# carltonyfakhry/geneticsCRE

Measured on AMD Instinct MI355X. Metric: path_x_permutation_scores_per_sec, higher is better.
Workload: dtype u32

## Files before the change

### geneticscre_amd/csrc/gcre_host.h

```cpp
#pragma once
#include "../../include/gcre_hip.h"
#include "gcre_kernels.h"

#include <dlfcn.h>
#include <rccl/rccl.h>

#include <algorithm>
#include <array>
#include <atomic>
#include <chrono>
#include <cmath>
#include <cstdio>
#include <cstdlib>
#include <cstring>
#include <limits>
#include <memory>
#include <mutex>
#include <condition_variable>
#include <string>
#include <unordered_map>
#include <thread>
#include <functional>
#include <deque>
#include <vector>
// ... 244 lines not shown
  int meet(uint64_t tag) {
    std::vector<float> none;
    return reduce(none, tag);
  }
  void fail() {
    std::lock_guard<std::mutex> lk(m);
    failed = true;
    cv.notify_all();
  }
};

struct gcre_ctx {
  Geometry g{};
  int device = 0;
  int top_k = 12;
  hipStream_t stream = nullptr;
  hipStream_t sel_stream = nullptr;
  hipEvent_t ev_sel = nullptr, ev_sel_done = nullptr;
  bool sel_async = true;
  hipStream_t insp_stream = nullptr;
  hipEvent_t ev_insp_done = nullptr;
  hipEvent_t ev_insp_main = nullptr;
  hipEvent_t ev_tail = nullptr;
  uint32_t* d_max_tot_b = nullptr;
  std::vector<JoinPlan>* ahead = nullptr;
  bool ahead_closed = false;
  bool ahead_on = true;
  SelectState h_sel{};
  std::string err;
  int last_code = GCRE_OK;
  bool quiet = false;
  bool have_table = false, have_perms = false;
  int64_t chunk_paths = int64_t(1) << 25;
  int null_blocks_per_cu = 12;
  int cus = 256;
  int64_t overlap_launches = 0;
  int64_t stepdown_launches = 0;
  int64_t clump_launches = 0;

  uint64_t* d_case_mask = nullptr;
  uint32_t* d_masks = nullptr;
  float* d_t32 = nullptr;
  double* d_dvt = nullptr;
  double* d_dmax = nullptr;
  double* d_dmaxn = nullptr;
  uint32_t* d_null = nullptr;
  uint32_t* d_mt = nullptr;
  bool mt_stale = false;
  int ieq_batch = 0;
  int ie_quad = 1;
  int ie_flagq = 1;
  int ie_zwide = 0;
  int ie_warm_items = 4;
  int exchange_tail = 0;
  int ie_warm_segs = 1024;
  int ie_small_join_tiles = 8;
  int ie_batch = 2;
  uint32_t* d_queue = nullptr;
  uint32_t* d_max_tot = nullptr;
  uint32_t* d_ladder = nullptr;
  uint32_t g00_rows = 0xffffffffu;
  int null_kernel = 0;
  int sparse_waves_per_cu = 32;
  int ie_prune = 1;
  uint64_t mask_epoch = 0;
  uint64_t obs_epoch = 0;
  bool insp_cache = false;
  ExchangeHub* hub = nullptr;
  ncclComm_t comm = nullptr;
  int64_t rccl_calls = 0;
  DevBuf<float> d_hub_null;
  int hub_level = 0, hub_round = 0;
  int win_k0 = 0, win_K = 0;
  int win_K_nominal = 0;

  ChunkBufs scratch;
  DevBuf<uint32_t> d_sel, d_small, d_chunk, d_rec_segs;
  DevBuf<uint64_t> d_wkey, d_doff, d_scan, d_excess, d_excess_b;
  DevBuf<uint32_t> d_wcases, d_wctrls, d_wrow0, d_wrow1;
  DevBuf<uint64_t> d_ie_timing;

  struct PlaneBuf { uint32_t* p; size_t bytes; };
  std::vector<PlaneBuf> plane_pool;
  std::unordered_map<uint64_t, const gcre_pathset*> live_sets;
  std::vector<gcre_uids*> live_uids;
  std::vector<gcre_gene_tally*> live_tallies;
  gcre_gene_tally* armed_tally = nullptr;
  gcre_gene_tally* pp_tally[6] = {nullptr, nullptr, nullptr, nullptr, nullptr, nullptr};
  std::vector<gcre_exceed*> live_exceeds;
  gcre_exceed* armed_exceed = nullptr;
  gcre_exceed* pp_exceed[6] = {nullptr, nullptr, nullptr, nullptr, nullptr, nullptr};
  std::vector<gcre_hits*> live_hits;
  gcre_hits* armed_hits = nullptr;
  gcre_hits* pp_hits[6] = {nullptr, nullptr, nullptr, nullptr, nullptr, nullptr};
  int64_t hits_launches = 0;
  uint64_t next_set_id = 0;
  size_t planes_out_max = (size_t)8 << 30;

  gcre_profile prof{};
  std::vector<std::pair<hipEvent_t, hipEvent_t>> ev_null, ev_stats;
  std::vector<hipEvent_t> ev_pool;
};

struct gcre_recipe {
  uint64_t a_id = 0, z_id = 0;
  uint64_t a_ver = 0, z_ver = 0;
// ... 136 lines not shown
```

### geneticscre_amd/csrc/gcre_host.hip

```cpp
#include "gcre_host.h"

namespace {

thread_local std::string g_create_error;

inline bool poison_fresh_planes() {
  static const bool on = std::getenv("GCRE_POISON") != nullptr && std::atoi(std::getenv("GCRE_POISON")) != 0;
  return on;
}
inline void poison_planes(void* p, size_t bytes) {
  if (!poison_fresh_planes() || !p) return;
  (void)hipDeviceSynchronize();
  (void)hipMemset(p, 0x5A, bytes);
  (void)hipDeviceSynchronize();
}

inline size_t tri(size_t t) { return t * (t + 1) / 2; }

template <typename Pred>
void pack_bits_host(const int32_t* data, int64_t nrow, int ncol, bool col_major, uint64_t* out, size_t stride, Pred pred) {
  const int W = (ncol + 63) / 64;
  if (nrow <= 0 || W <= 0) return;
  unsigned T = std::min<unsigned>(16u, std::max(1u, std::thread::hardware_concurrency()));
  if (const char* e = std::getenv("GCRE_PACK_THREADS")) T = (unsigned)std::max(1, std::atoi(e));
// ... 409 lines not shown
      });
      uint32_t run = 0;
      for (size_t k = 0; k < nkeys; k++)
        for (int t = 0; t < T; t++) {
          const uint32_t h = start[(size_t)t][k];
          start[(size_t)t][k] = run;
          run += h;
        }
      run_all([&](int t) {
        const Local& L = loc[(size_t)t];
        std::vector<uint32_t>& st = start[(size_t)t];
        for (size_t e = 0; e < L.part[q].size(); e++) segs[base + st[L.key[q][e]]++] = L.part[q][e];
      });
    } else {
      std::vector<SparseSeg> all;
      all.reserve(nq);
      for (const Local& L : loc) all.insert(all.end(), L.part[q].begin(), L.part[q].end());
      auto key_of = [&](const SparseSeg& x) { return u.h_location[x.row0] + ((int64_t)x.first + first - pi[x.row0]); };
      std::stable_sort(all.begin(), all.end(), [&](const SparseSeg& x, const SparseSeg& y) { return key_of(x) < key_of(y); });
      std::copy(all.begin(), all.end(), segs.begin() + (std::ptrdiff_t)base);
    }
    base += nq;
  }
  *nscored_out = (int64_t)n_scored;
}

void build_quads_host(const gcre_uids& u, const std::vector<SparseSeg>& segs, int64_t first, int64_t nscored, int64_t n_warm,
                      std::vector<uint32_t>& quads, int64_t* quad_begin_out) {
  const auto& pi = u.h_path_idx;
  const int64_t n = (int64_t)segs.size();
  quads.clear();
  int64_t quad_begin = -1;
  const int64_t qmax = ieq_quad_segs();
  quads.reserve((size_t)n / (size_t)std::max<int64_t>(1, (qmax + 1) / 2) + 16);
  auto key_of = [&](const SparseSeg& x) { return u.h_location[x.row0] + ((int64_t)x.first + first - pi[x.row0]); };
  int64_t i = 0;
  while (i < n) {
    if (i >= n_warm && quad_begin < 0) quad_begin = (int64_t)quads.size();
    const int64_t stop = i < n_warm ? n_warm : (i < nscored ? nscored : n);
    const int64_t k0 = key_of(segs[(size_t)i]);
    const uint32_t n0 = segs[(size_t)i].n;
    int64_t j = i + 1;
    while (j < stop && j < i + qmax && segs[(size_t)j].n == n0 && key_of(segs[(size_t)j]) == k0) j++;
    quads.push_back((uint32_t)i | ((uint32_t)(j - i - 1) << 30));
    i = j;
  }
  if (quad_begin < 0) quad_begin = (int64_t)quads.size();
  *quad_begin_out = quad_begin;
}

int64_t warm_segments(const gcre_ctx* c, int64_t nseg_scored, int nkt) {
  if (c->ie_warm_segs == 0) return 0;
  const int64_t warm_min = std::max<int64_t>(256, (int64_t)c->ie_warm_segs * 8 / std::max(nkt, 8));
  return std::min<int64_t>(nseg_scored, std::min<int64_t>(std::max<int64_t>(warm_min, nseg_scored / 1024),
                                                          std::max<int64_t>(256, nseg_scored / 8)));
}

int sparse_segments(gcre_ctx* c, const gcre_uids& u, int64_t first, int64_t count, int64_t score_b, int64_t score_e,
                    int64_t plane_b, int64_t plane_e, const SparseSeg** d_out, int64_t* nsegs, int64_t* nscored,
                    gcre_uids::SegCache** entry = nullptr) {
  plane_b = std::max(plane_b, first);
  plane_e = std::min(plane_e, first + count);
  for (auto& sc : u.seg_cache)
    if (sc.first == first && sc.count == count && sc.score_b == score_b && sc.score_e == score_e && sc.plane_b == plane_b &&
        sc.plane_e == plane_e) {
      *d_out = sc.d_segs;
      *nsegs = sc.nsegs;
      *nscored = sc.nscored;
      if (entry) *entry = &sc;
      return GCRE_OK;
    }
  std::vector<SparseSeg> segs;
  int64_t n_scored_i = 0;
  gcre_uids::Prefetch* pf = u.prefetch.get();
  if (pf && pf->th.joinable()) {
    HostTimer hw("prefetched tables: wait");
    pf->th.join();
  }
  if (pf && pf->ready && pf->first == first && pf->count == count && pf->score_b == score_b && pf->score_e == score_e &&
      pf->plane_b == plane_b && pf->plane_e == plane_e) {
    segs.swap(pf->segs);
    n_scored_i = pf->nscored;
    pf->ready = false;
    pf->quads_for_table = true;
  } else {
    HostTimer ht("sparse_segments");
    build_segments_host(u, first, count, score_b, score_e, plane_b, plane_e, segs, &n_scored_i);
  }
  const size_t n_scored = (size_t)n_scored_i;
  SparseSeg* d = nullptr;
  HIP_TRY(c, hipMalloc((void**)&d, std::max<size_t>(segs.size(), 1) * sizeof(SparseSeg)));
  if (!segs.empty())
    HIP_TRY(c, hipMemcpyAsync(d, segs.data(), segs.size() * sizeof(SparseSeg), hipMemcpyHostToDevice, c->stream));
  HIP_TRY(c, hipStreamSynchronize(c->stream));
  if (u.seg_cache.size() >= 64) {
    (void)hipFree(u.seg_cache.front().d_segs);
    if (u.seg_cache.front().d_quads) (void)hipFree(u.seg_cache.front().d_quads);
    u.seg_cache.erase(u.seg_cache.begin());
  }
  u.seg_cache.push_back({first, count, score_b, score_e, plane_b, plane_e, (int64_t)segs.size(), (int64_t)n_scored, d});
  if (c->g.method == 1 && c->ie_quad) u.seg_cache.back().h_segs = std::move(segs);
  if (entry) *entry = &u.seg_cache.back();
  *d_out = d;
  *nsegs = u.seg_cache.back().nsegs;
  *nscored = (int64_t)n_scored;
  return GCRE_OK;
}
// ... 1196 lines not shown
    ia.rec_lover = r0->lover.p;
    ia.rec_slot = r0->slot.p;
    ia.rec_over = r0->over.p;
    ia.rec_planes_a = R.rec_a->d_planes;
    ia.rec_planes_z = R.rec_z->d_planes;
    ia.rec_rows_a = (uint32_t)(R.rec_a->nrows * g.method);
    ia.rec_rows_z = (uint32_t)(R.rec_z->nrows * g.method);
    ia.rec_ga = R.rec_a->plane_groups;
    ia.rec_gz = R.rec_z->plane_groups;
    if (g.method == 1) {
      HIP_TRY(c, c->d_rec_segs.reserve((size_t)std::max<int64_t>(ia.nsegs, 1) * kRecSegWords));
      HIP_TRY(c, launch_fill_rec_segs(ia.segs, ia.nsegs, r0->row0.p, r0->rowz.p, r0->linfo.p, r0->lover.p, r0->slot.p, r0->tot.p,
                                      c->d_rec_segs.p, R.st));
      ia.rec_segs = c->d_rec_segs.p;
    }
  }
  ia.t32 = c->d_t32;
  ia.d64 = c->d_dmax;
  ia.ladder = c->d_ladder;
  ia.ladder_stride = g.TD;
  ia.lad_mode = !C.scored ? 1 : (c->ie_prune ? 0 : 2);
  ia.g00_rows = c->g00_rows;
  ia.null_bits = R.w_null;
  ia.planes_out = R.res_planes ? jp.res->d_planes : nullptr;
  ia.go = R.res_planes ? jp.res->plane_groups : 0;
  ia.out_first = cb;
  ia.score_begin = (uint32_t)C.s0;
  ia.score_end = (uint32_t)C.s1;
  ia.score_segs = (uint32_t)*nseg_scored;
  ia.nkt = R.nkt_sp;
  ia.K = g.K;
  ia.mt_rows = (uint32_t)(64 * g.Wp + 1);
  ia.zoff = (uint32_t)(64 * g.Wp) << 8;
  return GCRE_OK;
}

int launch_ie_slices(JoinRun& R, const ChunkRun& C, IeArgs& ia, int planes, int64_t nseg_scored,
                     gcre_uids::SegCache* seg_entry, int64_t ie_tile_factor, bool* quad_ran) {
  gcre_ctx* c = R.c;
  const JoinPlan& jp = R.jp;
  const Geometry& g = R.g;
  hipStream_t st = R.st;
  const int64_t n = C.n;
  ia.seg_begin = 0;
  ia.seg_end = ia.nsegs;
  if (c->d_ladder && ia.lad_mode == 0) {
    int64_t n_warm = warm_segments(c, nseg_scored, R.nkt_sp);
    if (jp.exchange && R.exchanges_done < jp.exchanges && R.P > 0)
      n_warm = std::min(n_warm, std::max<int64_t>(64, (int64_t)((double)n_warm * (double)(R.se - R.sb) / (double)R.P) + 1));
    if (c->ie_warm_segs == 0) n_warm = 0;
    IeArgs wa = ia;
    wa.seg_end = n_warm;
    wa.waves_per_xcd = spread_waves(wa.waves_per_xcd, n_warm * R.nkt_sp, c->ie_warm_items);
    if (n_warm > 0) HIP_TRY(c, launch_null_ie(wa, g.method, planes, true, st));
    ia.seg_begin = n_warm;
  }
  if (ia.seg_begin >= ia.seg_end) return GCRE_OK;
  ia.queue = c->d_queue;
  ia.batch = c->ie_batch;
  bool quad = false;
  if (g.method == 1 && c->d_ladder && c->ie_quad && !ia.planes_out && seg_entry &&
      ensure_quads(c, *R.u, *seg_entry, ia.seg_begin) == GCRE_OK) {
    const int64_t nq = seg_entry->nquads - seg_entry->quad_begin;
    const int64_t qmax = ieq_quad_segs();
    quad = nq > 0 && ((ia.seg_end - ia.seg_begin) * 4 >= nq * (4 + (qmax - 1)) || c->ie_quad == 2);
    if (std::getenv("GCRE_HOST_TIMING"))
      std::fprintf(stderr, "[host] quads: %lld segments in %lld quads (%.2f per quad), %lld joined paths, quad form %s\n",
                   (long long)(ia.seg_end - ia.seg_begin), (long long)nq, (double)(ia.seg_end - ia.seg_begin) / (double)std::max<int64_t>(nq, 1),
                   (long long)n, quad ? "on" : "off");
    if (quad) {
      ia.quads = seg_entry->d_quads;
      ia.quad_begin = seg_entry->quad_begin;
      ia.quad_end = seg_entry->nquads;
      const uint64_t z_units = (uint64_t)ia.rowsz * (uint64_t)ia.gz;
      ia.flagq = (c->ie_flagq && (uint64_t)ia.mt_rows * 256u < (1ull << 31)) ? 1u : 0u;
      ia.z_wide = (c->ie_zwide || z_units >= (1ull << 22)) ? 1u : 0u;
      ia.z_tile_units = ia.z_wide ? 0u : (uint32_t)z_units;
      ia.batch = c->ieq_batch > 0 ? c->ieq_batch : std::max(1, c->ie_batch * 2);
      const int wq = std::min(c->sparse_waves_per_cu, ieq_max_waves_per_cu(planes, ia.gz, ia.rec_slot != nullptr, ia.z_wide != 0u));
      ia.waves_per_xcd = spread_waves(xcd_waves(c, wq), n * ie_tile_factor, 128);
    }
  }
  while (((ia.nsegs - ia.seg_begin) / ia.batch + 1) * (int64_t)ia.nkt > (int64_t)0xf0000000ll) ia.batch *= 2;
  const bool pruned = c->d_ladder && ia.lad_mode == 0;
  const int n_slices = (pruned && jp.exchange) ? std::max(1, jp.exchanges - R.exchanges_done) : 1;
  const int64_t r_b = quad ? ia.quad_begin : ia.seg_begin, r_e = quad ? ia.quad_end : ia.seg_end;
  int64_t lo = r_b;
  for (int sl = 0; sl < n_slices && lo < r_e; sl++) {
    int64_t hi = r_e;
    if (sl + 1 < n_slices) {
      const int m = std::min(n_slices - 1, c->exchange_tail < 0 ? n_slices / 2 : c->exchange_tail), head = n_slices - m;
      const double end = sl >= head ? (double)(sl - head + 2) / (double)(m + 1) : std::ldexp(1.0 / (double)(m + 1), -(head - 1 - sl));
      hi = std::min(r_e, std::max(lo + 1, r_b + (int64_t)((double)(r_e - r_b) * end)));
    }
    if (pruned && jp.exchange)
      if (int rc = exchange_now(R)) return rc;
    IeArgs sa2 = ia;
    if (quad) { sa2.quad_begin = lo; sa2.quad_end = hi; }
    else { sa2.seg_begin = lo; sa2.seg_end = hi; }
    HIP_TRY(c, hipMemsetAsync(sa2.queue, 0, 8 * 16 * 4, st));
    if (quad) HIP_TRY(c, launch_null_ie_quad(sa2, planes, st));
    else HIP_TRY(c, launch_null_ie(sa2, g.method, planes, c->d_ladder == nullptr, st));
    lo = hi;
  }
  if (quad) R.prof->ie_quad_launches++;
  *quad_ran = quad;
  return GCRE_OK;
// ... 67 lines not shown
    if (cb > C.sg->b || C.sg != &R.segs.front()) {
      R.recipe_broken = true;
      R.hint_broke_late = true;
    }
    if (ci) ci->inspected = false;
    *end = ChunkEnd::kRedoHint;
    return GCRE_OK;
  }
  if (ci && !C.hit) {
    std::memcpy(ci->flags, C.flags, sizeof C.flags);
    ci->flags_valid = true;
  }
  if (R.mode == kInspect) {
    if (C.sel_begun && !C.sel_done) {
      HIP_TRY(c, hipStreamSynchronize(C.sel_on));
      if (int rc = finish_selection(R, C)) return rc;
    }
    *end = ChunkEnd::kInspected;
    return GCRE_OK;
  }
  const int64_t nseg_est = std::max<int64_t>(uids_in(*R.u, cb, n), 1);
  if (c->null_kernel == 0 && C.scored && ie_dearer(g, R.nkt_sp, R.have_p0, row_max(c, jp.p0), nseg_est, n, n_list)) {
    R.res_planes_ok = false;
    *end = C.partial ? ChunkEnd::kResplit : ChunkEnd::kPricedOut;
    return GCRE_OK;
  }
  if (!C.scored && !(R.res_planes && cb < R.pl_e && cb + n > R.pl_b)) {
    *end = ChunkEnd::kNotNeeded;
    return GCRE_OK;
  }
  const int planes = counter_planes(max_tot);
  IeArgs ia{};
  int64_t nseg_scored = 0;
  gcre_uids::SegCache* seg_entry = nullptr;
  if (int rc = fill_ie_args(R, C, ia, &nseg_scored, &seg_entry)) return rc;
  R.prof->null_row_loads += ((R.have_p0 ? 0.0 : (double)row_max(c, jp.p0) * g.method * (double)nseg_est) + (double)n_list) * R.nkt_sp;
  const int wpc = std::min(c->sparse_waves_per_cu, ie_max_waves_per_cu(g.method, planes, ia.gz, ia.planes_out != nullptr, ia.rec_slot != nullptr));
  const int64_t ie_tile_factor = std::min(std::max(R.nkt_sp * c->ie_small_join_tiles / 8, 1), R.nkt_sp);
  ia.waves_per_xcd = spread_waves(xcd_waves(c, wpc), n * ie_tile_factor, 32);
  R.prof->inspect_ms += std::chrono::duration<double, std::milli>(std::chrono::steady_clock::now() - ti0).count();
  ia.stats = R.mode == kLaunch ? R.w_null + g.Kpad : R.flagblk + kFlagLookupTiles;
  if (jp.exceed || R.mode == kCount) {
    C.ie = ia;
    C.ie_planes = planes;
    C.ie_segs = nseg_scored;
    C.ie_ok = true;
    if (R.mode == kCount) {
      *end = ChunkEnd::kScored;
      return GCRE_OK;
    }
  }
  const bool timing = std::getenv("GCRE_IE_TIMING") != nullptr;
  if (timing) {
    HIP_TRY(c, c->d_ie_timing.reserve(12));
    HIP_TRY(c, hipMemsetAsync(c->d_ie_timing.p, 0, 96, st));
    ia.timing = c->d_ie_timing.p;
  }
  if (C.sel_begun && C.sel_on == st)
    if (int rc = finish_selection(R, C)) return rc;
  hipEvent_t n0 = get_event(c), n1 = get_event(c);
  bool quad = false;
  HIP_TRY(c, hipEventRecord(n0, st));
  if (int rc = launch_ie_slices(R, C, ia, planes, nseg_scored, seg_entry, ie_tile_factor, &quad)) return rc;
  HIP_TRY(c, hipEventRecord(n1, st));
  if (C.sel_begun && !C.sel_done) {
    const auto tw0 = std::chrono::steady_clock::now();
    HIP_TRY(c, hipStreamSynchronize(C.sel_on));
    R.select_wait_ms += std::chrono::duration<double, std::milli>(std::chrono::steady_clock::now() - tw0).count();
    if (int rc = finish_selection(R, C)) return rc;
  }
  if (timing && R.mode != kLaunch)
    if (int rc = print_ie_timing(R, C, ia, quad)) return rc;
  R.ev_null->emplace_back(n0, n1);
  if (C.scored) {
    R.prof->null_kernel_launches++;
    R.prof->null_alg_bytes += alg_bytes(R, cb + C.s0, C.s1 - C.s0);
  }
  R.prof->ie_launches++;
  R.prof->ie_overlap_lists += C.flags[kFlagOverlapLists];
  R.ie_stat_pending = true;
  R.ie_ran = true;
  *end = ChunkEnd::kScored;
  return GCRE_OK;
}

int score_chunk_sparse(JoinRun& R, ChunkRun& C, ChunkEnd* end) {
  gcre_ctx* c = R.c;
  const JoinPlan& jp = R.jp;
  const gcre_uids& u = *R.u;
  const Geometry& g = R.g;
  hipStream_t st = R.st;
  ChunkBufs& b = *C.b;
  ChunkInsp* ci = C.ci;
  const int64_t cb = C.cb, n = C.n;
  if (int rc = ensure_lists(c, jp.p0)) return rc;
  if (int rc = ensure_lists(c, jp.p1)) return rc;
  const uint32_t zoff = (uint32_t)(64 * g.Wp) << 8;
  const int64_t nl = n * g.method;
  HIP_TRY(c, c->d_doff.reserve((size_t)nl + 1));
  HIP_TRY(c, c->d_scan.reserve((size_t)(nl + 1023) / 1024 + 2));
  HIP_TRY(c, launch_scan_u32_u64(b.dcnt.p, nl, c->d_doff.p, c->d_scan.p, st));
  uint32_t max_tot = 0;
  uint64_t n_delta = 0;
  HIP_TRY(c, hipMemcpyAsync(&max_tot, R.flagblk + kFlagMaxTot, 4, hipMemcpyDeviceToHost, st));
  HIP_TRY(c, hipMemcpyAsync(&n_delta, c->d_doff.p + nl, 8, hipMemcpyDeviceToHost, st));
  HIP_TRY(c, hipStreamSynchronize(st));
  if (C.hit) max_tot = ci->flags[kFlagMaxTot];
  else if (ci) { ci->flags[kFlagMaxTot] = max_tot; ci->flags_valid = true; }
// ... 266 lines not shown
  return (hipGetDeviceCount(&n) == hipSuccess && n > 0) ? n : 0;
}

const char* gcre_last_error(const gcre_ctx* ctx) { return ctx ? ctx->err.c_str() : g_create_error.c_str(); }

gcre_ctx* gcre_create(int method, int n_cases, int n_ctrls, int iterations, int device) {
  if ((method != 1 && method != 2) || n_cases <= 0 || n_ctrls <= 0 || iterations < 0) {
    g_create_error = "assertion: need method in {1,2}, num_cases > 0, num_ctrls > 0, iterations >= 0";
    return nullptr;
  }
  int ndev = 0;
  if (hipGetDeviceCount(&ndev) != hipSuccess || ndev <= 0) {
    g_create_error = "no HIP device: libgcre_hip has no CPU fallback";
    return nullptr;
  }
  if (device < 0 || device >= ndev) {
    g_create_error = "device index out of range";
    return nullptr;
  }
  hipDeviceProp_t prop;
  if (hipSetDevice(device) != hipSuccess || hipGetDeviceProperties(&prop, device) != hipSuccess) {
    g_create_error = "cannot select HIP device";
    return nullptr;
  }
  if (std::strncmp(prop.gcnArchName, "gfx950", 6) != 0) {
    g_create_error = std::string("kernels are built for gfx950 only, device is ") + prop.gcnArchName;
    return nullptr;
  }
  auto* c = new gcre_ctx();
  c->device = device;
  (void)hipDeviceGetAttribute(&c->cus, hipDeviceAttributeMultiprocessorCount, device);
  Geometry& g = c->g;
  g.method = method;
  g.n = n_cases + n_ctrls;
  g.n_cases = n_cases;
  g.W = (g.n + 63) / 64;
  g.Wp = ((g.W + 3) / 4) * 4;
  g.S = g.Wp * method;
  g.K = iterations;
  g.Kpad = ((iterations + kPermTileMax - 1) / kPermTileMax) * kPermTileMax;
  g.TD = 64 * g.Wp + 1;
  c->win_k0 = 0;
  c->win_K = g.K;
  if (const char* e = std::getenv("GCRE_QUIET")) c->quiet = std::atoi(e) != 0;
  g_launch_trace = std::getenv("GCRE_LAUNCH_TRACE") != nullptr;
  if (const char* e = std::getenv("GCRE_CHUNK_PATHS")) c->chunk_paths = std::max<long long>(64, std::atoll(e));
  if (const char* e = std::getenv("GCRE_NULL_BLOCKS_PER_CU")) c->null_blocks_per_cu = std::max(1, std::atoi(e));
  if (const char* e = std::getenv("GCRE_NULL_KERNEL"))
    c->null_kernel = !std::strcmp(e, "dense") ? 1 : !std::strcmp(e, "sparse") ? 2 : !std::strcmp(e, "ie") ? 3 : 0;
  if (const char* e = std::getenv("GCRE_IE_PRUNE")) c->ie_prune = std::atoi(e) != 0;
  if (const char* e = std::getenv("GCRE_EXCHANGE_TAIL")) c->exchange_tail = std::min(std::max(std::atoi(e), -1), 64);
  if (const char* e = std::getenv("GCRE_IE_WARM")) c->ie_warm_segs = std::min(std::max(std::atoi(e), 0), 1 << 20);
  if (const char* e = std::getenv("GCRE_IE_WARM_ITEMS")) c->ie_warm_items = std::min(std::max(std::atoi(e), 1), 64);
  if (const char* e = std::getenv("GCRE_IE_SJT")) c->ie_small_join_tiles = std::atoi(e);
  if (const char* e = std::getenv("GCRE_IE_BATCH")) c->ie_batch = std::min(std::max(std::atoi(e), 1), 4096);
  if (const char* e = std::getenv("GCRE_IEQ_BATCH")) c->ieq_batch = std::max(0, std::atoi(e));
  if (const char* e = std::getenv("GCRE_IE_QUAD")) c->ie_quad = std::min(std::max(std::atoi(e), 0), 2);
  if (const char* e = std::getenv("GCRE_IE_FLAGQ")) c->ie_flagq = std::atoi(e) != 0;
  if (const char* e = std::getenv("GCRE_IE_ZWIDE")) c->ie_zwide = std::atoi(e) != 0;
  if (const char* e = std::getenv("GCRE_PLANES_OUT_MAX_MB")) c->planes_out_max = (size_t)std::max(0ll, std::atoll(e)) << 20;
  if (const char* e = std::getenv("GCRE_SPARSE_WAVES_PER_CU")) c->sparse_waves_per_cu = std::max(1, std::atoi(e));

  bool ok = hipStreamCreateWithFlags(&c->stream, hipStreamNonBlocking) == hipSuccess;
  ok = ok && hipStreamCreateWithFlags(&c->sel_stream, hipStreamNonBlocking) == hipSuccess;
  ok = ok && hipStreamCreateWithFlags(&c->insp_stream, hipStreamNonBlocking) == hipSuccess;
  ok = ok && hipEventCreateWithFlags(&c->ev_insp_done, hipEventDisableTiming) == hipSuccess;
  ok = ok && hipEventCreateWithFlags(&c->ev_insp_main, hipEventDisableTiming) == hipSuccess;
  ok = ok && hipEventCreateWithFlags(&c->ev_tail, hipEventDisableTiming) == hipSuccess;
  if (const char* e = std::getenv("GCRE_AHEAD")) c->ahead_on = std::atoi(e) != 0;
  ok = ok && hipEventCreateWithFlags(&c->ev_sel, hipEventDisableTiming) == hipSuccess;
  ok = ok && hipEventCreateWithFlags(&c->ev_sel_done, hipEventDisableTiming) == hipSuccess;
  if (const char* e = std::getenv("GCRE_SELECT_STREAM")) c->sel_async = std::atoi(e) != 0;
  ok = ok && hipMalloc((void**)&c->d_case_mask, (size_t)g.Wp * 8) == hipSuccess;
  ok = ok && hipMalloc((void**)&c->d_max_tot, kFlagWords * 4) == hipSuccess;
  ok = ok && hipMalloc((void**)&c->d_max_tot_b, kFlagWords * 4) == hipSuccess;
  ok = ok && hipMalloc((void**)&c->d_queue, 8 * 16 * 4) == hipSuccess;
  if (ok && g.Kpad > 0) {
    ok = hipMalloc((void**)&c->d_masks, (size_t)2 * g.Wp * g.Kpad * 4) == hipSuccess;
    ok = ok && hipMalloc((void**)&c->d_null, (size_t)g.Kpad * 4) == hipSuccess;
    ok = ok && hipMemsetAsync(c->d_masks, 0, (size_t)2 * g.Wp * g.Kpad * 4, c->stream) == hipSuccess;
  }
  if (ok) {
    std::vector<uint64_t> cm((size_t)g.Wp, 0);
    for (int k = 0; k < n_cases; k++) cm[(size_t)k / 64] |= uint64_t(1) << (k % 64);
    ok = hipMemcpy(c->d_case_mask, cm.data(), cm.size() * 8, hipMemcpyHostToDevice) == hipSuccess;
  }
  if (!ok) {
    g_create_error = "device allocation failed in gcre_create";
    gcre_destroy(c);
    return nullptr;
  }
  return c;
}

void gcre_destroy(gcre_ctx* c) {
  if (!c) return;
  (void)hipSetDevice(c->device);
  if (c->stream) (void)hipStreamSynchronize(c->stream);
  if (c->insp_stream) (void)hipStreamSynchronize(c->insp_stream);
  drop_ahead(c);
  while (!c->live_uids.empty()) free_uids(c->live_uids.back());
  while (!c->live_tallies.empty()) gcre_gene_tally_free(c->live_tallies.back());
  while (!c->live_exceeds.empty()) gcre_exceed_free(c->live_exceeds.back());
  while (!c->live_hits.empty()) gcre_hits_free(c->live_hits.back());
  {
    std::vector<const gcre_pathset*> sets;
// ... 1026 lines not shown
```

### geneticscre_amd/csrc/gcre_ie.hip

```cpp
#include "gcre_ie_common.h"

namespace gcre {



template <int M, int L>
__global__ __launch_bounds__(64 * kIeWaves) __attribute__((amdgpu_waves_per_eu(M == 1 ? 4 : 2))) void k_null_ie(const IeArgs a) {
  static_assert(L % 4 == 0 && L >= 8 && L <= 16, "planes come in groups of 4");
  const int lane = threadIdx.x & 63;
  const int wave = __builtin_amdgcn_readfirstlane(threadIdx.x >> 6);
  const int xcd = blockIdx.x & 7;
  const i64 wi = (i64)(blockIdx.x >> 3) * kIeWaves + wave;
  const i64 wx = a.waves_per_xcd;
  const i64 slices = 8 * wx;
  const u32 lane4 = (u32)lane * 4u;
  __shared__ u32 gmax_lds[kIeWaves][32 * 64];
  u32* scr = gmax_lds[wave] + lane;
#pragma unroll
  for (int q = 0; q < 32; q++) scr[q * 64] = 0u;

  const SparseSeg GCRE_CONSTANT* segs = (const SparseSeg GCRE_CONSTANT*)a.segs;
  const u64 GCRE_CONSTANT* loff0 = (const u64 GCRE_CONSTANT*)a.loff0;
  const u32 GCRE_CONSTANT* lidx0 = (const u32 GCRE_CONSTANT*)a.lidx0;

  int cur_kt = -1;
  __amdgpu_buffer_rsrc_t mt = __builtin_amdgcn_make_buffer_rsrc((void*)a.mt, 0, 0x7fffffff, 0x00020000);

  auto flush = [&]() {
    if (cur_kt < 0) return;
    u32* out = a.null_bits + (size_t)cur_kt * 2048 + lane * 32;
    for (int q = 0; q < 32; q++) {
      const u32 own = scr[q * 64];
      if (own != 0u) {
        atomicMax(out + q, own);
        scr[q * 64] = 0u;
      }
    }
  };

  auto to_counts = [&](const u32 (&C)[L], u32 (&R)[16]) {
#pragma unroll
    for (int l = 0; l < 16; l++) R[l] = (l < L) ? C[l] : 0u;
    transpose16(R);
  };
  auto finish_m1 = [&](const u32 (&C)[L], u32 total) {
    u32 R[16];
    to_counts(C, R);
    const u32* diag_g = (const u32*)a.t32 + sp_diag_offset(total);
    u32 v[32], o[32];
#pragma unroll
    for (int j = 0; j < 16; j++) {
      v[j] = diag_g[R[j] & 0xffffu];
      v[j + 16] = diag_g[R[j] >> 16];
    }
#pragma unroll
    for (int q = 0; q < 32; q++) o[q] = scr[q * 64];
#pragma unroll
    for (int q = 0; q < 32; q++)
      if (v[q] > o[q]) scr[q * 64] = v[q];
  };

  auto finish_m2 = [&](const u32 (&Cp)[L], const u32 (&Cn)[L], u32 tp, u32 tn) {
    u32 Rp[16], Rn[16];
    to_counts(Cp, Rp);
    to_counts(Cn, Rn);
    const double* dp = a.d64 + sp_diag_offset(tp);
    const double* dn = a.d64 + sp_diag_offset(tn);
#pragma unroll
    for (int g0 = 0; g0 < 16; g0 += 4) {
      double sp[8], sn[8];
      u32 o[8];
#pragma unroll
      for (int k = 0; k < 4; k++) {
        sp[k] = dp[Rp[g0 + k] & 0xffffu];
        sn[k] = dn[Rn[g0 + k] & 0xffffu];
        sp[k + 4] = dp[Rp[g0 + k] >> 16];
        sn[k + 4] = dn[Rn[g0 + k] >> 16];
        o[k] = scr[(g0 + k) * 64];
        o[k + 4] = scr[(g0 + k + 16) * 64];
      }
#pragma unroll
      for (int k = 0; k < 8; k++) {
        float f = (float)(sp[k] + sn[k]);
        f = (f > 0.0f) ? f : 0.0f;
        const u32 v = __float_as_uint(f);
        const int q = (k < 4) ? g0 + k : g0 + k - 4 + 16;
        if (v > o[k]) scr[q * 64] = v;
      }
    }
  };

  auto load_planes = [&](u32 (&P)[L], const u32* planes, u32 unit, int groups) {
    const u32x4* src = (const u32x4*)(planes + (u64)unit * 256u) + lane;
#pragma unroll
    for (int j = 0; j < L / 4; j++) {
      u32x4 v = {0u, 0u, 0u, 0u};
      if (j < groups) v = src[j * 64];
      P[4 * j + 0] = v.x;
      P[4 * j + 1] = v.y;
      P[4 * j + 2] = v.z;
      P[4 * j + 3] = v.w;
    }
  };

  for (int step = 0; step < a.nkt; step++) {
    const i64 item = (i64)xcd * a.nkt * wx + wi + (i64)step * wx;
    const int kt = (int)(item / slices);
    const i64 sl = item % slices;
    if (kt != cur_kt) {
      flush();
      cur_kt = kt;
      mt = __builtin_amdgcn_make_buffer_rsrc((void*)(a.mt + (size_t)kt * a.mt_rows * 64), 0, 0x7fffffff, 0x00020000);
    }
    for (i64 sidx = a.seg_begin + sl; sidx < a.seg_end; sidx += slices) {
      const u32 row0 = segs[sidx].row0;
      const u32 first = segs[sidx].first;
      const u32 npaths = segs[sidx].n;
      const u32 qv = first + (((u32)lane < npaths) ? (u32)lane : 0u);
      u32 infov[M], lovv[M];
#pragma unroll
      for (int h = 0; h < M; h++) {
        infov[h] = a.linfo[(u64)qv * M + h];
        lovv[h] = a.lover[(u64)qv * M + h];
      }
      const u32 rzv = a.rowz[qv];
      u32 zunit[M];
#pragma unroll
      for (int h = 0; h < M; h++) {
        const u32 hz = (M == 2 && (rzv >> 31)) ? (u32)(1 - h) : (u32)h;
        zunit[h] = ((u32)kt * (u32)a.rowsz + (rzv & 0x7fffffffu) * (u32)M + hz) * (u32)a.gz;
      }
      u32 ttv[M];
#pragma unroll
      for (int h = 0; h < M; h++) ttv[h] = a.tot[(u64)qv * M + h];
      u32 lv[M][8];
#pragma unroll
      for (int h = 0; h < M; h++) {
        const u32x4* lp = (const u32x4*)(a.dlist + ((u64)qv * M + h) * 8u);
        const u32x4 e0 = lp[0], e1 = lp[1];
        lv[h][0] = e0.x; lv[h][1] = e0.y; lv[h][2] = e0.z; lv[h][3] = e0.w;
        lv[h][4] = e1.x; lv[h][5] = e1.y; lv[h][6] = e1.z; lv[h][7] = e1.w;
      }

      auto stream = [&](u32 (&P)[L], const u32 GCRE_CONSTANT* list, u64 p, u64 e) {
        u32 x[16];
        for (; p + 16 <= e; p += 16) {
          load16(x, mt, lane4, *(const u32x16 GCRE_CONSTANT*)(list + p));
          add16<L>(P, x);
        }
        for (; p < e; p += 4) {
          const u32x4 offs = *(const u32x4 GCRE_CONSTANT*)(list + p);
          u32 y4[4];
#pragma unroll
          for (int j = 0; j < 4; j++) y4[j] = __builtin_amdgcn_raw_buffer_load_b32(mt, lane4, offs[j], 0);
          add4<L>(P, y4);
        }
      };

      u32 B[M][L];
#pragma unroll
      for (int h = 0; h < M; h++) {
        const u64 r = (u64)row0 * M + h;
        if (a.planes0) {
          load_planes(B[h], a.planes0, (u32)(((u64)kt * (u64)a.rows0 + r) * (u64)a.g0), a.g0);
        } else if (a.rec_slot) {
          const u32 ra = a.rec_row0[row0], rzr = a.rec_rowz[row0], rz = rzr & 0x7fffffffu, rinfo = a.rec_linfo[r];
          const u32 hz = (M == 2 && (rzr >> 31)) ? (u32)(1 - h) : (u32)h;
          u32 ZR[L], S[L];
          load_planes(B[h], a.rec_planes_a, (u32)(((u64)kt * (u64)a.rec_rows_a + (u64)ra * M + h) * (u64)a.rec_ga), a.rec_ga);
          load_planes(ZR, a.rec_planes_z, (u32)(((u64)kt * (u64)a.rec_rows_z + (u64)rz * M + hz) * (u64)a.rec_gz), a.rec_gz);
#pragma unroll
          for (int l = 0; l < L; l++) S[l] = 0u;
          const u32 rlen = linfo_len(rinfo);
          stream(S, (const u32 GCRE_CONSTANT*)(a.rec_slot + r * 8u), 0, 8);
          if (rlen > 8u) stream(S, (const u32 GCRE_CONSTANT*)(a.rec_over + a.rec_lover[r]), 0, (u64)(rlen - 8u));
          u32 cy = 0u, bw = 0u;
#pragma unroll
          for (int l = 0; l < L; l++) {
            const u32 zl = linfo_overlap(rinfo) ? ZR[l] : S[l];
            const u32 sl_ = linfo_overlap(rinfo) ? S[l] : 0u;
            const u32 s1_ = B[h][l] ^ zl ^ cy;
            cy = maj3(B[h][l], zl, cy);
            B[h][l] = s1_ ^ sl_ ^ bw;
            bw = maj3(~s1_, sl_, bw);
          }
        } else {
#pragma unroll
          for (int l = 0; l < L; l++) B[h][l] = 0u;
          stream(B[h], lidx0, loff0[r], loff0[r + 1]);
        }
      }

      for (u32 t = 0; t < npaths; t++) {
        const u32 q = first + t;
        u32 C[M][L];
#pragma unroll
        for (int h = 0; h < M; h++) {
          const u32 r0 = rdlane(infov[h], t);
          const u32 len = linfo_len(r0);
          const bool overlap = linfo_overlap(r0);
          u32 offs[8], y[8];
#pragma unroll
          for (int j = 0; j < 8; j++) offs[j] = rdlane(lv[h][j], t);
#pragma unroll
          for (int j = 0; j < 8; j++) y[j] = __builtin_amdgcn_raw_buffer_load_b32(mt, lane4, offs[j], 0);
          u32 Z[L];
          if (overlap) {
            load_planes(Z, a.planesz, rdlane(zunit[h], t), a.gz);
          } else {
#pragma unroll
            for (int l = 0; l < L; l++) Z[l] = 0u;
          }
          u32 c0, a0, c1, a1, c2, a2, d0, b0;
          csa(c0, a0, y[0], y[1], y[2]);
          csa(c1, a1, y[3], y[4], y[5]);
          csa(c2, a2, a0, a1, y[6]);
          const u32 s0 = a2 ^ y[7], c3 = a2 & y[7];
          csa(d0, b0, c0, c1, c2);
          const u32 s1 = b0 ^ c3, d1 = b0 & c3;
          u32 S[L];
          S[0] = s0; S[1] = s1; S[2] = d0 ^ d1; S[3] = d0 & d1;
#pragma unroll
          for (int l = 4; l < L; l++) S[l] = 0u;
          if (len > 8u) stream(S, (const u32 GCRE_CONSTANT*)(a.dover + rdlane(lovv[h], t)), 0, (u64)(len - 8u));
          if (overlap) {
            u32 cy = 0u, bw = 0u;
#pragma unroll
            for (int l = 0; l < L; l++) {
              const u32 s1_ = B[h][l] ^ Z[l] ^ cy;
              cy = maj3(B[h][l], Z[l], cy);
              C[h][l] = s1_ ^ S[l] ^ bw;
              bw = maj3(~s1_, S[l], bw);
            }
          } else {
            u32 cy = 0u;
#pragma unroll
            for (int l = 0; l < L; l++) {
              C[h][l] = B[h][l] ^ S[l] ^ cy;
              cy = maj3(B[h][l], S[l], cy);
            }
          }
        }
        if (a.planes_out) {
#pragma unroll
          for (int h = 0; h < M; h++) {
            const u64 rh = ((u64)a.out_first + q) * M + h;
            u32x4* dst = (u32x4*)(a.planes_out + (((u64)cur_kt * (u64)a.rows_out + rh) * (u64)a.go) * 256u) + lane;
#pragma unroll
            for (int j = 0; j < 4; j++) {
              if (j < a.go) {
                u32x4 v = {0u, 0u, 0u, 0u};
                if (4 * j < L) v = u32x4{C[h][(4 * j) % L], C[h][(4 * j + 1) % L], C[h][(4 * j + 2) % L], C[h][(4 * j + 3) % L]};
                dst[j * 64] = v;
              }
            }
          }
        }
        if (q < a.score_begin || q >= a.score_end) continue;
        if constexpr (M == 1) {
          finish_m1(C[0], rdlane(ttv[0], t));
        } else {
          finish_m2(C[0], C[M - 1], rdlane(ttv[0], t), rdlane(ttv[M - 1], t));
        }
      }
    }
  }
  flush();
}


template <int L, int GZ, bool OUT, bool REC>
__global__ __launch_bounds__(64 * kIeWaves) __attribute__((amdgpu_waves_per_eu(L <= 12 ? 4 : 3))) void k_null_ie_m1(const IeArgs a) {
  constexpr int LP = (L + 3) / 4 * 4;
  static_assert(L >= 8 && L <= 16 && GZ >= 2 && 4 * GZ <= LP, "planes come in groups of 4");
  __shared__ u32 nmax_lds[kIeWaves][32 * 64];
  const int lane = threadIdx.x & 63;
  const int wave = __builtin_amdgcn_readfirstlane(threadIdx.x >> 6);
  const u32 lane4 = (u32)lane * 4u;
  u32* nm = nmax_lds[wave] + lane;
#pragma unroll
  for (int q = 0; q < 32; q++) nm[q * 64] = 0u;
  const SparseSeg GCRE_CONSTANT* segs = (const SparseSeg GCRE_CONSTANT*)a.segs;
  const char* k_planesz = (const char*)(((u64)(u32)__builtin_amdgcn_readfirstlane((int)(u32)((u64)a.planesz >> 32)) << 32) |
                                        (u64)(u32)__builtin_amdgcn_readfirstlane((int)(u32)(u64)a.planesz));

  int cur_kt = -1;
  u32 valid = 0u;
  u32 lad_base = (a.lad_mode == 0) ? 0u : (u32)(kLadderLevels - 1 + a.lad_mode) * (u32)a.ladder_stride;
  const u32 lad_keep = (u32)kLadderLevels * (u32)a.ladder_stride;
  bool dirty = false;
  u32 n_slow = 0u;
#ifdef GCRE_IE_TIMING
  u64 tm[6] = {0, 0, 0, 0, 0, 0};
  const u64 tm_begin = __builtin_amdgcn_s_memtime();
#define GCRE_TM_MARK(var) __builtin_amdgcn_s_waitcnt(0); const u64 var = __builtin_amdgcn_s_memtime()
#define GCRE_TM_ADD(i, t1, t0) tm[i] += (t1) - (t0)
#else
#define GCRE_TM_MARK(var)
#define GCRE_TM_ADD(i, t1, t0)
#endif
  __amdgpu_buffer_rsrc_t mt = __builtin_amdgcn_make_buffer_rsrc((void*)a.mt, 0, 0x7fffffff, 0x00020000);

  auto exchange = [&]() {
    u32* out = a.null_bits + (size_t)cur_kt * 2048 + lane * 32;
    __amdgpu_buffer_rsrc_t nb = __builtin_amdgcn_make_buffer_rsrc((void*)(a.null_bits + (size_t)cur_kt * 2048), 0, 8192, 0x00020000);
    u32x4 g4[8];
#pragma unroll
    for (int j = 0; j < 8; j++) g4[j] = __builtin_amdgcn_raw_buffer_load_b128(nb, (u32)lane * 128u + (u32)j * 16u, 0, 16 );
    u32 lo = 0xffffffffu;
#pragma unroll
    for (int q = 0; q < 32; q++) {
      const u32 g = g4[q >> 2][q & 3];
      const u32 own = nm[q * 64];
      if (dirty && own > g) atomicMax(out + q, own);
      const u32 v = own > g ? own : g;
      if ((valid >> q) & 1u) lo = v < lo ? v : lo;
    }
    dirty = false;
    u32 theta = __builtin_amdgcn_readfirstlane(wave_min_u32(lo));
    if (theta == 0xffffffffu) theta = 0u;
    int j = (int)(__uint_as_float(theta) * (float)kLadderPerUnit);
    j = j < 0 ? 0 : (j > kLadderLevels - 1 ? kLadderLevels - 1 : j);
    lad_base = (u32)j * (u32)a.ladder_stride;
  };
  auto flush_tile = [&]() {
    if (cur_kt >= 0) {
      u32* out = a.null_bits + (size_t)cur_kt * 2048 + lane * 32;
#pragma unroll 8
      for (int q = 0; q < 32; q++) {
        const u32 own = nm[q * 64];
        if (own != 0u) {
          atomicMax(out + q, own);
          nm[q * 64] = 0u;
        }
      }
    }
    dirty = false;
  };

  __shared__ u32 wq_state[kIeWaves][8];
  WorkQueue wq;
  wq.st = wq_state[wave];
  wq.init(a.queue, (u32)((a.seg_end - a.seg_begin + a.batch - 1) / a.batch), (u32)a.nkt);
  {
    wq.select(blockIdx.x & 7u);
  }
  u32 ticket = wq.take(lane);
  int since = 0, period = 1;
  for (;;) {
    const u32 work = __builtin_amdgcn_readfirstlane(ticket);
    const u32 q_n = wq.get(2);
    if (work >= q_n) {
// ... 488 lines not shown
    GCRE_IE_M2(EXPR)                                               \
  }

__global__ __launch_bounds__(256) void k_fill_rec_segs(const SparseSeg* segs, i64 nsegs, const u32* r_row0, const u32* r_rowz,
                                                       const u32* r_linfo, const u32* r_lover, const u32* r_slot, const u32* r_tot,
                                                       u32* out) {
  const i64 t = (i64)blockIdx.x * blockDim.x + threadIdx.x;
  const i64 sidx = t >> 2;
  const int part = (int)(t & 3);
  if (sidx >= nsegs) return;
  const u32 row0 = segs[sidx].row0;
  u32* o = out + sidx * kRecSegWords;
  if (part == 0) {
    o[0] = r_row0[row0];
    o[1] = r_rowz[row0];
  } else if (part == 1) {
    u32 info = r_linfo[row0];
    u32 need = 3u;
    if (r_tot) {
      const u32 t = r_tot[row0];
      need = t < 16u ? 0u : (t < 256u ? 1u : (t < 4096u ? 2u : 3u));
    }
    o[2] = linfo_with_groups(info, need);
    o[3] = r_lover[row0];
  } else {
    const u32x4 v = *(const u32x4*)(r_slot + (u64)row0 * 8u + (part - 2) * 4);
    *(u32x4*)(o + 4 + (part - 2) * 4) = v;
  }
}

hipError_t launch_fill_rec_segs(const SparseSeg* segs, int64_t nsegs, const uint32_t* r_row0, const uint32_t* r_rowz,
                                const uint32_t* r_linfo, const uint32_t* r_lover, const uint32_t* r_slot, const uint32_t* r_tot,
                                uint32_t* out, hipStream_t stream) {
  if (nsegs == 0) return hipSuccess;
  const i64 blocks = (nsegs * 4 + 255) / 256;
  hipLaunchKernelGGL(k_fill_rec_segs, dim3((unsigned)blocks), dim3(256), 0, stream, segs, nsegs, r_row0, r_rowz, r_linfo, r_lover,
                     r_slot, r_tot, out);
  return hipGetLastError();
}

hipError_t launch_null_ie(const IeArgs& a, int method, int planes, bool general, hipStream_t stream) {
  const dim3 grid((unsigned)(8 * a.waves_per_xcd / kIeWaves));
  const dim3 block(64 * kIeWaves);
  if (method == 1 && !general) {
    const int gz = a.gz;
    const bool out = a.planes_out != nullptr;
    const bool rec = a.rec_slot != nullptr;
#define GCRE_LAUNCH(LL, GG, OO, RR) hipLaunchKernelGGL((k_null_ie_m1<LL, GG, OO, RR>), grid, block, 0, stream, a)
    GCRE_IE_M1(GCRE_LAUNCH)
#undef GCRE_LAUNCH
  } else if (method == 2 && !general) {
    return launch_null_ie_m2(a, planes, stream);
  } else {
#define GCRE_LAUNCH(MM, LL) hipLaunchKernelGGL((k_null_ie<MM, LL>), grid, block, 0, stream, a)
    GCRE_IE_GEN(GCRE_LAUNCH)
#undef GCRE_LAUNCH
  }
  return hipGetLastError();
}

int ie_max_waves_per_cu(int method, int planes, int gz, bool out, bool rec) {
  int blocks = 0;
  hipError_t e = hipSuccess;
  if (method == 1) {
#define GCRE_OCC(LL, GG, OO, RR) e = hipOccupancyMaxActiveBlocksPerMultiprocessor(&blocks, k_null_ie_m1<LL, GG, OO, RR>, 64 * kIeWaves, 0)
    GCRE_IE_M1(GCRE_OCC)
#undef GCRE_OCC
  } else {
    return ie2_max_waves_per_cu(planes, gz, out, rec);
  }
  if (e != hipSuccess || blocks < 1) blocks = 1;
  return blocks * kIeWaves;
}

template <int L>
__global__ __launch_bounds__(256) void k_build_planes(const u32* mt_all, u32 mt_rows, int nkt, const u64* loff,
                                                      const u32* lidx, i64 nrowhalves, int groups, u32* planes) {
  const int lane = threadIdx.x & 63;
  const i64 wave = (i64)blockIdx.x * 4 + __builtin_amdgcn_readfirstlane(threadIdx.x >> 6);
  const i64 nwaves = (i64)gridDim.x * 4;
  const u32 lane4 = (u32)lane * 4u;
  const u64 GCRE_CONSTANT* off = (const u64 GCRE_CONSTANT*)loff;
  const u32 GCRE_CONSTANT* list = (const u32 GCRE_CONSTANT*)lidx;
  const i64 items = nrowhalves * nkt;
  for (i64 it = wave; it < items; it += nwaves) {
    const i64 w = it / nrowhalves;
    const i64 rr = it - w * nrowhalves;
    __amdgpu_buffer_rsrc_t mt = __builtin_amdgcn_make_buffer_rsrc((void*)(mt_all + (size_t)w * mt_rows * 64), 0, 0x7fffffff, 0x00020000);
    u32 P[L];
#pragma unroll
    for (int l = 0; l < L; l++) P[l] = 0u;
    u64 p = off[rr];
    const u64 e = off[rr + 1];
    u32 x[16];
    for (; p + 16 <= e; p += 16) {
      load16(x, mt, lane4, *(const u32x16 GCRE_CONSTANT*)(list + p));
      add16<L>(P, x);
    }
    for (; p < e; p += 4) {
      const u32x4 offs = *(const u32x4 GCRE_CONSTANT*)(list + p);
      u32 y[4];
#pragma unroll
      for (int j = 0; j < 4; j++) y[j] = __builtin_amdgcn_raw_buffer_load_b32(mt, lane4, offs[j], 0);
      add4<L>(P, y);
    }
    u32x4* dst = (u32x4*)(planes + (((u64)w * (u64)nrowhalves + (u64)rr) * (u64)groups) * 256u) + lane;
// ... 156 lines not shown
```

Baseline: 9521 billion.

## Restructure warm IE kernel work split and merge block maxima before atomics

The general k_null_ie kernel, used for warm segments, now hands each block a contiguous chunk of segments per key tile, with one segment per wave, instead of strided slices. Its flush first reduces the per-wave LDS maxima across the block and compares them against the global null bits, so it issues fewer atomicMax operations. The warm-segment count divisor moves from 1024 to a tunable 4096, which shrinks the warm phase for large segment counts. Optional timing instrumentation is added; the kernel now uses two block barriers per flush and rejects launches where waves_per_xcd is not a multiple of kIeWaves.

```diff
diff --git a/geneticscre_amd/csrc/gcre_host.h b/geneticscre_amd/csrc/gcre_host.h
--- a/geneticscre_amd/csrc/gcre_host.h
+++ b/geneticscre_amd/csrc/gcre_host.h
@@ -320,6 +320,7 @@
   int ie_flagq = 1;
   int ie_zwide = 0;
   int ie_warm_items = 4;
+  int ie_warm_div = 4096;
   int exchange_tail = 0;
   int ie_warm_segs = 1024;
   int ie_small_join_tiles = 8;
diff --git a/geneticscre_amd/csrc/gcre_host.hip b/geneticscre_amd/csrc/gcre_host.hip
--- a/geneticscre_amd/csrc/gcre_host.hip
+++ b/geneticscre_amd/csrc/gcre_host.hip
@@ -485,7 +485,7 @@
 int64_t warm_segments(const gcre_ctx* c, int64_t nseg_scored, int nkt) {
   if (c->ie_warm_segs == 0) return 0;
   const int64_t warm_min = std::max<int64_t>(256, (int64_t)c->ie_warm_segs * 8 / std::max(nkt, 8));
-  return std::min<int64_t>(nseg_scored, std::min<int64_t>(std::max<int64_t>(warm_min, nseg_scored / 1024),
+  return std::min<int64_t>(nseg_scored, std::min<int64_t>(std::max<int64_t>(warm_min, nseg_scored / c->ie_warm_div),
                                                           std::max<int64_t>(256, nseg_scored / 8)));
 }
 
@@ -1788,7 +1788,18 @@
     IeArgs wa = ia;
     wa.seg_end = n_warm;
     wa.waves_per_xcd = spread_waves(wa.waves_per_xcd, n_warm * R.nkt_sp, c->ie_warm_items);
+    if (wa.timing) wa.timing += 12;
     if (n_warm > 0) HIP_TRY(c, launch_null_ie(wa, g.method, planes, true, st));
+    if (n_warm > 0 && wa.timing && R.mode != kLaunch) {
+      uint64_t tw[7] = {0};
+      HIP_TRY(c, hipMemcpyAsync(tw, wa.timing, sizeof tw, hipMemcpyDeviceToHost, st));
+      HIP_TRY(c, hipStreamSynchronize(st));
+      const double waves = 8.0 * wa.waves_per_xcd;
+      std::fprintf(stderr, "[ie warm timing] level %d paths %lld segments %lld x %d tiles, waves %.0f: per-wave kcycles prologue %.1f paths to counts %.1f "
+                   "transpose+look-ups %.1f flush %.1f (%.2f flushes) total %.1f, slowest wave %.1f\n", R.u->path_length, (long long)n,
+                   (long long)n_warm, wa.nkt, waves, tw[0] / waves / 1e3, tw[1] / waves / 1e3, tw[2] / waves / 1e3, tw[3] / waves / 1e3,
+                   (double)tw[4] / waves, tw[5] / waves / 1e3, tw[6] / 1e3);
+    }
     ia.seg_begin = n_warm;
   }
   if (ia.seg_begin >= ia.seg_end) return GCRE_OK;
@@ -1962,8 +1973,8 @@
   }
   const bool timing = std::getenv("GCRE_IE_TIMING") != nullptr;
   if (timing) {
-    HIP_TRY(c, c->d_ie_timing.reserve(12));
-    HIP_TRY(c, hipMemsetAsync(c->d_ie_timing.p, 0, 96, st));
+    HIP_TRY(c, c->d_ie_timing.reserve(24));
+    HIP_TRY(c, hipMemsetAsync(c->d_ie_timing.p, 0, 192, st));
     ia.timing = c->d_ie_timing.p;
   }
   if (C.sel_begun && C.sel_on == st)
@@ -2336,6 +2347,7 @@
   if (const char* e = std::getenv("GCRE_EXCHANGE_TAIL")) c->exchange_tail = std::min(std::max(std::atoi(e), -1), 64);
   if (const char* e = std::getenv("GCRE_IE_WARM")) c->ie_warm_segs = std::min(std::max(std::atoi(e), 0), 1 << 20);
   if (const char* e = std::getenv("GCRE_IE_WARM_ITEMS")) c->ie_warm_items = std::min(std::max(std::atoi(e), 1), 64);
+  if (const char* e = std::getenv("GCRE_IE_WARM_DIV")) c->ie_warm_div = std::min(std::max(std::atoi(e), 1), 1 << 30);
   if (const char* e = std::getenv("GCRE_IE_SJT")) c->ie_small_join_tiles = std::atoi(e);
   if (const char* e = std::getenv("GCRE_IE_BATCH")) c->ie_batch = std::min(std::max(std::atoi(e), 1), 4096);
   if (const char* e = std::getenv("GCRE_IEQ_BATCH")) c->ieq_batch = std::max(0, std::atoi(e));
diff --git a/geneticscre_amd/csrc/gcre_ie.hip b/geneticscre_amd/csrc/gcre_ie.hip
--- a/geneticscre_amd/csrc/gcre_ie.hip
+++ b/geneticscre_amd/csrc/gcre_ie.hip
@@ -2,7 +2,13 @@
 
 namespace gcre {
 
-
+#ifdef GCRE_IE_TIMING
+#define GCRE_TM_MARK(var) __builtin_amdgcn_s_waitcnt(0); const u64 var = __builtin_amdgcn_s_memtime()
+#define GCRE_TM_ADD(i, t1, t0) tm[i] += (t1) - (t0)
+#else
+#define GCRE_TM_MARK(var)
+#define GCRE_TM_ADD(i, t1, t0)
+#endif
 
 template <int M, int L>
 __global__ __launch_bounds__(64 * kIeWaves) __attribute__((amdgpu_waves_per_eu(M == 1 ? 4 : 2))) void k_null_ie(const IeArgs a) {
@@ -10,9 +16,10 @@
   const int lane = threadIdx.x & 63;
   const int wave = __builtin_amdgcn_readfirstlane(threadIdx.x >> 6);
   const int xcd = blockIdx.x & 7;
-  const i64 wi = (i64)(blockIdx.x >> 3) * kIeWaves + wave;
-  const i64 wx = a.waves_per_xcd;
-  const i64 slices = 8 * wx;
+  const i64 bi = (i64)(blockIdx.x >> 3);
+  const i64 bx = a.waves_per_xcd / kIeWaves;
+  const i64 cpt = (a.seg_end - a.seg_begin + kIeWaves - 1) / kIeWaves;
+  const i64 chunks = cpt * a.nkt;
   const u32 lane4 = (u32)lane * 4u;
   __shared__ u32 gmax_lds[kIeWaves][32 * 64];
   u32* scr = gmax_lds[wave] + lane;
@@ -25,17 +32,44 @@
 
   int cur_kt = -1;
   __amdgpu_buffer_rsrc_t mt = __builtin_amdgcn_make_buffer_rsrc((void*)a.mt, 0, 0x7fffffff, 0x00020000);
+#ifdef GCRE_IE_TIMING
+  u64 tm[6] = {0, 0, 0, 0, 0, 0};
+  const u64 tm_begin = __builtin_amdgcn_s_memtime();
+#endif
 
   auto flush = [&]() {
     if (cur_kt < 0) return;
-    u32* out = a.null_bits + (size_t)cur_kt * 2048 + lane * 32;
-    for (int q = 0; q < 32; q++) {
-      const u32 own = scr[q * 64];
-      if (own != 0u) {
-        atomicMax(out + q, own);
-        scr[q * 64] = 0u;
-      }
-    }
+    GCRE_TM_MARK(tf0);
+    __syncthreads();
+    const u32 slot0 = (u32)wave * 512u + (u32)lane * 8u;
+    __amdgpu_buffer_rsrc_t nb = __builtin_amdgcn_make_buffer_rsrc((void*)(a.null_bits + (size_t)cur_kt * 2048), 0, 8192, 0x00020000);
+    const u32x4 g0 = __builtin_amdgcn_raw_buffer_load_b128(nb, slot0 * 4u, 0, 16 );
+    const u32x4 g1 = __builtin_amdgcn_raw_buffer_load_b128(nb, slot0 * 4u + 16u, 0, 16 );
+    u32* out = a.null_bits + (size_t)cur_kt * 2048 + slot0;
+    u32* cell = &gmax_lds[0][0] + (slot0 & 31u) * 64u + (slot0 >> 5);
+    u32 own[8];
+#pragma unroll
+    for (int j = 0; j < 8; j++) {
+      u32 m = 0u;
+#pragma unroll
+      for (int w = 0; w < kIeWaves; w++) {
+        const u32 v = cell[w * 32 * 64 + j * 64];
+        m = v > m ? v : m;
+        cell[w * 32 * 64 + j * 64] = 0u;
+      }
+      own[j] = m;
+    }
+#pragma unroll
+    for (int j = 0; j < 8; j++) {
+      const u32 g = j < 4 ? g0[j & 3] : g1[j & 3];
+      if (own[j] > g) atomicMax(out + j, own[j]);
+    }
+    __syncthreads();
+    GCRE_TM_MARK(tf1);
+    GCRE_TM_ADD(3, tf1, tf0);
+#ifdef GCRE_IE_TIMING
+    tm[4] += 1;
+#endif
   };
 
   auto to_counts = [&](const u32 (&C)[L], u32 (&R)[16]) {
@@ -103,16 +137,17 @@
     }
   };
 
-  for (int step = 0; step < a.nkt; step++) {
-    const i64 item = (i64)xcd * a.nkt * wx + wi + (i64)step * wx;
-    const int kt = (int)(item / slices);
-    const i64 sl = item % slices;
+  const i64 c_end = (i64)(xcd + 1) * chunks / 8;
+  for (i64 c = (i64)xcd * chunks / 8 + bi; c < c_end; c += bx) {
+    const int kt = (int)(c / cpt);
     if (kt != cur_kt) {
       flush();
       cur_kt = kt;
       mt = __builtin_amdgcn_make_buffer_rsrc((void*)(a.mt + (size_t)kt * a.mt_rows * 64), 0, 0x7fffffff, 0x00020000);
     }
-    for (i64 sidx = a.seg_begin + sl; sidx < a.seg_end; sidx += slices) {
+    const i64 sidx = a.seg_begin + (c - (i64)kt * cpt) * kIeWaves + wave;
+    if (sidx < a.seg_end) {
+      GCRE_TM_MARK(ts0);
       const u32 row0 = segs[sidx].row0;
       const u32 first = segs[sidx].first;
       const u32 npaths = segs[sidx].n;
@@ -191,7 +226,10 @@
         }
       }
 
+      GCRE_TM_MARK(ts1);
+      GCRE_TM_ADD(0, ts1, ts0);
       for (u32 t = 0; t < npaths; t++) {
+        GCRE_TM_MARK(tp0);
         const u32 q = first + t;
         u32 C[M][L];
 #pragma unroll
@@ -256,16 +294,26 @@
             }
           }
         }
+        GCRE_TM_MARK(tp1);
+        GCRE_TM_ADD(1, tp1, tp0);
         if (q < a.score_begin || q >= a.score_end) continue;
         if constexpr (M == 1) {
           finish_m1(C[0], rdlane(ttv[0], t));
         } else {
           finish_m2(C[0], C[M - 1], rdlane(ttv[0], t), rdlane(ttv[M - 1], t));
         }
+        GCRE_TM_MARK(tp2);
+        GCRE_TM_ADD(2, tp2, tp1);
       }
     }
   }
   flush();
+#ifdef GCRE_IE_TIMING
+  tm[5] = __builtin_amdgcn_s_memtime() - tm_begin;
+  if (a.timing && lane == 0)
+    for (int i = 0; i < 6; i++) atomicAdd((unsigned long long*)a.timing + i, (unsigned long long)tm[i]);
+  if (a.timing && lane == 0) atomicMax((unsigned long long*)a.timing + 6, (unsigned long long)tm[5]);
+#endif
 }
 
 
@@ -293,11 +341,6 @@
 #ifdef GCRE_IE_TIMING
   u64 tm[6] = {0, 0, 0, 0, 0, 0};
   const u64 tm_begin = __builtin_amdgcn_s_memtime();
-#define GCRE_TM_MARK(var) __builtin_amdgcn_s_waitcnt(0); const u64 var = __builtin_amdgcn_s_memtime()
-#define GCRE_TM_ADD(i, t1, t0) tm[i] += (t1) - (t0)
-#else
-#define GCRE_TM_MARK(var)
-#define GCRE_TM_ADD(i, t1, t0)
 #endif
   __amdgpu_buffer_rsrc_t mt = __builtin_amdgcn_make_buffer_rsrc((void*)a.mt, 0, 0x7fffffff, 0x00020000);
 
@@ -892,6 +935,7 @@
   } else if (method == 2 && !general) {
     return launch_null_ie_m2(a, planes, stream);
   } else {
+    if (a.waves_per_xcd < kIeWaves || a.waves_per_xcd % kIeWaves != 0) return hipErrorInvalidValue;
 #define GCRE_LAUNCH(MM, LL) hipLaunchKernelGGL((k_null_ie<MM, LL>), grid, block, 0, stream, a)
     GCRE_IE_GEN(GCRE_LAUNCH)
 #undef GCRE_LAUNCH
```

After: 9738 billion (median of 6 runs). 1.02x the previous value.
